# uci-cbcl/esm-efficient

Measured on AMD Instinct MI355X. Metric: residues/sec ESM2-650M fwd, 50k packed tokens; % bf16 MFMA peak; 1/2/4/8 GPU, higher is better.
Workload: dtype bf16

## Files before the change

esm-efficient_amd/csrc/forward.hip:

```cpp
#include "launch.h"

using namespace esme;

namespace {

#define ESME_TRY(call) do { if (const int rc_ = (call)) return rc_; } while (0)

enum Mode { FAST, HALF, EXACT };
const char* const kWho[] = {"forward", "forward_half", "forward_exact"};
constexpr float kLog2e = 1.4426950408889634f;

struct Arena {
    char* base;
    int64_t off;
    char* take(int64_t bytes) {
        const int64_t o = off;
        off += (bytes + 255) & ~int64_t(255);
        return base ? base + o : nullptr;
    }
};

struct Ws {
    char* xs;
    char* h;
// ... 83 lines not shown
    layout(mode, m, T, &w, workspace);
    const int Ep = m->phys_dim, E = m->embed_dim, H = m->heads, dp = m->head_pad;
    const int64_t Ea = (int64_t)H * dp;
    const int nblk = esme_hip_gemm_stats_blocks(T, Ep);
    const bool rot_fused = m->rotary && !m->qk_norm && (dp == 16 || dp == 32 || dp == 64) && Ea % 32 == 0;
    const bool qk_pair = half && m->half_qk_pair != 0;
    if (qk_pair && (m->qk_norm || !(dp == 16 || dp == 32 || dp == 64) || Ea % 128 != 0))
        ESME_FAIL(ESME_ERR_UNSUPPORTED, "forward_half: q/k pairs cover blocks without q/k LayerNorm, head dim 16 / 32 / 64, heads * head_pad a multiple of 128");
    const int ext = half && m->half_ext_n > 0 ? 64 : 0;
    const int64_t lo_off = (int64_t)Ep + ext;
    void* const xs = half ? w.xs : x;
    const int64_t ldxs = half ? 2 * (int64_t)Ep + ext : ldx;
    const int Kf = Ep + ext;
    const bool qp = m->attn_q_prescale && m->rotary && (dp == 64 || dp == 32) && Ea % 64 == 0 && (rot_fused || m->qk_norm);
    const float qs = m->softmax_scale * kLog2e;
    esme_attn_opts_t aopts{(int)sizeof(esme_attn_opts_t), 0, 0, 8.0f, 1, nullptr, qp ? 1 : 0, half ? 1 : 0};
    if (m->n_layers > 0) ESME_TRY(sequence_order(cu_lens, B, w.order, stream, &aopts.seq_order));
    const float* stats = w.sums;
    int stats_nblk = 1;
    if (half)
        ESME_TRY(esme_hip_stream_operand_guarded((const float*)x, ldx, xs, ldxs, lo_off, 1, m->layers[0].ps_attn, ext ? m->half_ext_sel : nullptr, m->half_ext_n,
                                                 ext ? Ep : 0, w.sums, m->half_col_absmax, T, Ep, stream));
    else if (m->n_layers > 0)
        ESME_TRY(esme_hip_row_sums(x, ldx, T, Ep, w.sums, stream));
    auto folded = [&](esme_gemm_fusion_t& f, const float* c1, const float* c2) {
        if (half) { f.f16 = 1; f.overflow_flag = m->half_overflow_flag; }
        ln_fields(f, m, stats, stats_nblk, c1, c2);
    };
    auto residual = [&](const void* a, int64_t lda, const void* wt, const void* bias, int K, float* stats_out, const float* s_in, const float* s_out, int guard_row) {
        esme_gemm_fusion_t f{};
        f.stats_out = stats_out;
        if (half) {
            f.f16 = 1; f.pair_off = lo_off;
            if (ext) { f.ext_sel = m->half_ext_sel; f.ext_n = m->half_ext_n; f.ext_off = Ep; }
            f.pair_scale_in = s_in; f.pair_scale_out = s_out;
            if (m->half_col_absmax) f.col_absmax = m->half_col_absmax + (int64_t)guard_row * Ep;
        }
        return esme_hip_gemm_bf16_fused(a, lda, wt, bias, xs, ldxs, xs, ldxs, T, Ep, K, ESME_EPI_RESIDUAL, m->alpha, &f, stream);
    };
    for (int i = 0; i < m->n_layers; ++i) {
        const esme_layer_weights_t& L = m->layers[i];
        esme_gemm_fusion_t fu{};
        folded(fu, L.qkv_c1, L.qkv_c2);
        char* q = w.qkv; char* k = w.qkv + Ea * 2; char* v = w.qkv + 2 * Ea * 2;
        if (qk_pair && L.half_qk_pair) {
            fu.pair_off = 3 * Ea; fu.pair_cols = (int)(2 * Ea);
            if (m->rotary) rotary_fields(fu, m, m->cos32, m->sin32, pos);
            ESME_TRY(esme_hip_gemm_bf16_fused(xs, ldxs, L.qkv_w, nullptr, nullptr, 0, w.qkv, 5 * Ea, T, (int)(3 * Ea), Kf, ESME_EPI_NONE, 1.0f, &fu, stream));
            ESME_TRY(esme_hip_attn_varlen_fwd_qkpair_f16(q, k, v, 5 * Ea, 3 * Ea, w.attn, Ea, cu_lens, B, T, H, dp, max_len, m->softmax_scale, aopts.seq_order, stream));
        } else {
            uint32_t* const gq = half && m->half_qk_sumsq ? m->half_qk_sumsq + (int64_t)i * 2 * H : nullptr;
            if (rot_fused) { rotary_fields(fu, m, m->cos, m->sin, pos); fu.qk_sumsq = gq; }
            if (qp && rot_fused) { fu.q_scale = qs; fu.q_cols = (int)Ea; }
            ESME_TRY(esme_hip_gemm_bf16_fused(xs, ldxs, L.qkv_w, nullptr, nullptr, 0, w.qkv, 3 * Ea, T, (int)(3 * Ea), Kf, ESME_EPI_NONE, 1.0f, &fu, stream));
            if (m->qk_norm) {
                if (!half) ESME_TRY(esme_hip_qk_norm_rotary_scaled(q, k, 3 * Ea, L.lnq_w, L.lnk_w, L.lnq_b, L.lnk_b, m->ln_eps, m->cos, m->sin, pos, T, H, dp, m->table_len, qp ? qs : 1.0f, stream));
                else if (qp) ESME_TRY(esme_hip_qk_norm_rotary_f16_scaled(q, k, 3 * Ea, L.lnq_w, L.lnk_w, L.lnq_b, L.lnk_b, m->ln_eps, m->cos, m->sin, pos, T, H, dp, m->table_len, qs, gq, stream));
                else ESME_TRY(esme_hip_qk_norm_rotary_f16_guarded(q, k, 3 * Ea, L.lnq_w, L.lnk_w, L.lnq_b, L.lnk_b, m->ln_eps, m->cos, m->sin, pos, T, H, dp, m->table_len, gq, stream));
            } else if (m->rotary && !rot_fused) {
                ESME_TRY((half ? esme_hip_rotary_varlen_f16 : esme_hip_rotary_varlen)(q, k, 3 * Ea, m->cos, m->sin, pos, T, H, dp, m->table_len, stream));
            }
            ESME_TRY(esme_hip_attn_varlen_fwd_opts(q, k, v, 3 * Ea, w.attn, Ea, cu_lens, B, T, H, dp, max_len, m->softmax_scale, &aopts, stream));
        }
        ESME_TRY(residual(w.attn, Ea, L.out_w, L.out_b, (int)Ea, w.part_b, L.ps_attn_inv, L.ps_ffn, 2 * i + 1));
        stats = w.part_b; stats_nblk = nblk;
        esme_gemm_fusion_t fup{};
        folded(fup, L.up_c1, L.up_c2);
        ESME_TRY(esme_hip_gemm_bf16_fused(xs, ldxs, L.up_w, nullptr, nullptr, 0, w.mid, m->ffn_dim, T, m->swiglu ? 2 * m->ffn_dim : m->ffn_dim, Kf,
                                          m->swiglu ? ESME_EPI_SWIGLU : ESME_EPI_GELU, 1.0f, &fup, stream));
// ... 3 lines not shown
    if (half)
        return esme_hip_layernorm_split_checked(xs, ldxs, 2, lo_off, m->final_ln_w, m->final_ln_b, pair, ld_pair, Ep, rep32, ld_rep, T, E, m->ln_eps, m->half_overflow_flag, stream);
    ESME_TRY(esme_hip_layernorm(x, ldx, m->final_ln_w, m->final_ln_b, x, ldx, T, E, m->ln_eps, stream));
    if (!logits) return ESME_OK;
    ESME_CHECK_ARG(m->head_dense_w && m->head_ln_w && m->head_final_w && m->vocab > 0 && ld_logits >= m->vocab, "forward: LM head weights missing");
    ESME_TRY(esme_hip_gemm_bf16(x, ldx, m->head_dense_w, m->head_dense_b, nullptr, 0, w.head, Ep, T, Ep, Ep, ESME_EPI_GELU, 1.0f, stream));
    ESME_TRY(esme_hip_layernorm(w.head, Ep, m->head_ln_w, m->head_ln_b, w.head, Ep, T, E, m->ln_eps, stream));
    return esme_hip_gemm_bf16(w.head, Ep, m->head_final_w, m->head_final_b, nullptr, 0, logits, ld_logits, T, m->vocab, Ep, ESME_EPI_NONE, 1.0f, stream);
}

}

extern "C" int64_t esme_hip_forward_workspace_bytes(const esme_model_desc_t* m, int64_t T) { return workspace_bytes(FAST, m, T); }
extern "C" int64_t esme_hip_forward_half_workspace_bytes(const esme_model_desc_t* m, int64_t T) { return workspace_bytes(HALF, m, T); }
extern "C" int64_t esme_hip_forward_exact_workspace_bytes(const esme_model_desc_t* m, int64_t T) { return workspace_bytes(EXACT, m, T); }

extern "C" int esme_hip_forward(const esme_model_desc_t* m, void* x, int64_t ldx, const int32_t* cu_lens, int B, int64_t T,
                                int max_len, const int32_t* pos, void* workspace, int64_t ws_bytes, void* logits,
                                int64_t ld_logits, void* stream) {
    ESME_PROLOGUE(FAST, m, x, ldx, cu_lens, B, T, max_len, pos, workspace, ws_bytes, nullptr, 0);
    return forward_folded(FAST, m, x, ldx, cu_lens, B, T, max_len, pos, workspace, logits, ld_logits, nullptr, 0, nullptr, 0, stream);
}

extern "C" int esme_hip_forward_half(const esme_model_desc_t* m, const float* x32, int64_t ld32, const int32_t* cu_lens, int B, int64_t T,
                                     int max_len, const int32_t* pos, void* workspace, int64_t ws_bytes, void* pair, int64_t ld_pair,
                                     float* rep32, int64_t ld_rep, void* stream) {
    ESME_PROLOGUE(HALF, m, x32, ld32, cu_lens, B, T, max_len, pos, workspace, ws_bytes, pair, ld_pair);
    return forward_folded(HALF, m, const_cast<float*>(x32), ld32, cu_lens, B, T, max_len, pos, workspace, nullptr, 0, pair, ld_pair, rep32, ld_rep, stream);
}

// ... 44 lines not shown
```

esm-efficient_amd/esme/_hip.py:

```python
from __future__ import annotations

import ctypes
import os
import threading
from ctypes import POINTER, Structure, c_char_p, c_float, c_int, c_int64, c_void_p
from typing import Optional

import torch

_LIB_NAME = 'libesme_hip.so'
_LIB_PATH = os.environ.get('ESME_HIP_LIB') or os.path.join(os.path.dirname(os.path.abspath(__file__)), _LIB_NAME)
ABI_VERSION = 10

EPI_NONE, EPI_GELU, EPI_RESIDUAL, EPI_SWIGLU = 0, 1, 2, 3


class GemmFusion(Structure):
    _fields_ = [('ln_partial', c_void_p), ('ln_nblk', c_int), ('ln_dim', c_int), ('ln_eps', c_float), ('ln_c1', c_void_p), ('ln_c2', c_void_p), ('stats_out', c_void_p),
                ('cos', c_void_p), ('sin', c_void_p), ('pos', c_void_p),
                ('head_dim', c_int), ('max_len', c_int), ('rot_cols', c_int), ('resid32', c_void_p), ('ld32', c_int64), ('q_scale', c_float), ('q_cols', c_int),
                ('w_k', c_int), ('pair_off', c_int64), ('c32', c_void_p), ('ldc32', c_int64), ('f16', c_int),
                ('pair_scale_in', c_void_p), ('pair_scale_out', c_void_p),
                ('ext_sel', c_void_p), ('ext_n', c_int), ('ext_off', c_int64), ('pair_cols', c_int), ('overflow_flag', c_void_p),
                ('col_absmax', c_void_p), ('qk_sumsq', c_void_p)]


class GemmOpts(Structure):
# ... 8 lines not shown
class LayerWeights(Structure):
    _fields_ = [(n, c_void_p) for n in ('qkv_w', 'qkv_c1', 'qkv_c2', 'out_w', 'out_b', 'up_w', 'up_c1', 'up_c2',
                                        'down_w', 'down_b', 'lnq_w', 'lnk_w', 'lnq_b', 'lnk_b',
                                        'ps_attn', 'ps_attn_inv', 'ps_ffn', 'ps_ffn_inv',
                                        'ln1_w', 'ln1_b', 'ln2_w', 'ln2_b', 'qkv_b', 'up_b')] + [('half_qk_pair', c_int), ('reserved_', c_int)]


class ModelDesc(Structure):
    _fields_ = ([(n, c_int) for n in ('struct_bytes', 'n_layers', 'embed_dim', 'phys_dim', 'heads', 'head_dim', 'head_pad',
                                      'ffn_dim', 'vocab', 'swiglu', 'rotary', 'qk_norm', 'table_len')]
                + [('ln_eps', c_float), ('alpha', c_float), ('softmax_scale', c_float), ('attn_q_prescale', c_int),
                   ('layers', POINTER(LayerWeights))]
                + [(n, c_void_p) for n in ('final_ln_w', 'final_ln_b', 'head_dense_w', 'head_dense_b', 'head_ln_w',
                                           'head_ln_b', 'head_final_w', 'head_final_b', 'cos', 'sin')]
                + [('half_ext_n', c_int), ('half_ext_sel', c_void_p), ('half_qk_pair', c_int), ('half_overflow_flag', c_void_p),
                   ('cos32', c_void_p), ('sin32', c_void_p), ('half_col_absmax', c_void_p), ('half_qk_sumsq', c_void_p)])


SIGNATURES = {
    'esme_hip_abi_version': (c_int, []),
    'esme_hip_last_error': (c_char_p, []),
    'esme_hip_embed': (c_int, [c_void_p, c_void_p, c_void_p, c_int64, c_int, c_int, c_int, c_int, c_void_p]),
    'esme_hip_embed_positions': (c_int, [c_void_p, c_void_p, c_void_p, c_void_p, c_int, c_void_p, c_int64, c_int, c_int,
                                         c_int, c_int, c_void_p]),
    'esme_hip_seq_positions': (c_int, [c_void_p, c_int, c_int64, c_void_p, c_void_p, c_void_p]),
    'esme_hip_seq_order': (c_int, [c_void_p, c_int, c_void_p, c_void_p]),
    'esme_hip_layernorm': (c_int, [c_void_p, c_int64, c_void_p, c_void_p, c_void_p, c_int64, c_int64, c_int,
                                   c_float, c_void_p]),
    'esme_hip_rotary_varlen': (c_int, [c_void_p, c_void_p, c_int64, c_void_p, c_void_p, c_void_p, c_int64, c_int,
                                       c_int, c_int, c_void_p]),
    'esme_hip_rotary_varlen_f16': (c_int, [c_void_p, c_void_p, c_int64, c_void_p, c_void_p, c_void_p, c_int64, c_int,
# ... 956 lines not shown
```

esm-efficient_amd/esme/attention.py:

```python
from __future__ import annotations

import math
import os
from typing import NamedTuple, Optional

import torch
from torch import nn

from esme import _hip
from esme.nn import GELU, Derived, LayerNorm, Linear, pad_last, pad_rows, version_key
from esme.rotary import RotaryEmbedding

_ATTN_QP = os.environ.get('ESME_ATTN_QP', '1') != '0'


def _q_scale(head_dim: int) -> float:
    import numpy as np
    return float(np.float32(head_dim ** -0.5) * np.float32(1.4426950408889634))


class ForwardContext:
    __slots__ = ('pos', 'cos', 'sin', 'sums', 'part_a', 'part_b', 'fold', 'exact_attn', 'x32', 'order', 'scratch', 'f16', 'xs', 'plan', 'probe', 'ovf', 'cos32', 'sin32', 'guard', 'lora_x', 'observer',
                 'sites', 'fast_site')

    def __init__(self, pos, cos, sin, fold=False, exact_attn=False, f16=False, plan=None, cos32=None, sin32=None, probe=None, ovf=None, guard=None):
        self.pos, self.cos, self.sin = pos, cos, sin
        self.plan = plan
        self.probe = probe
        self.ovf = ovf
        self.guard = guard
        self.cos32, self.sin32 = cos32, sin32
        self.f16 = f16
        self.fold = fold
        self.exact_attn = exact_attn
        self.x32 = None
        self.xs = None
        self.order = None
        self.scratch = {}
        self.sums = None
        self.part_a = None
        self.part_b = None
        self.observer = None
        self.lora_x = None
        self.sites = None
        self.fast_site = None

    def fp32_stream(self, x32, x16, n_layers):
        self.x32 = x32
        self.sites = [{'resid32': x32, 'out': x16}] * (2 * n_layers)

    def pair_stream(self, xs, scales):
        self.xs = xs
        ext = self.plan.ext_sel if self.plan is not None else None
        col = self.guard.col if self.guard is not None else None
        self.sites = sites = []
        for i, ((_, a_inv), (f_rho, f_inv)) in enumerate(scales):
            nxt = scales[i + 1][0][0] if i + 1 < len(scales) else None
            for scale in ((a_inv, f_rho), (f_inv, nxt)):
                sites.append({'resid_pair': xs, 'pair_scale': scale, 'pair_ext': ext, 'col_absmax': col[len(sites) + 1] if col is not None else None})

# ... 313 lines not shown
        guard = ctx.guard if (f16 and ctx is not None) else None
        pair_ext = plan.ext_sel if plan is not None else None
        if stream is None and resid is not None:
            stream = {'resid': resid, 'out': out}
        if qk_pair:
            if self.pre_layernorm or d not in (16, 32, 64) or E % 128 != 0:
                raise NotImplementedError("precision='half' with q/k pairs covers ESM-2 / ESM-1 blocks with head dim 16 / 32 / 64 and a 128-aligned width")
            wf, _, c1, c2 = self._weights_qkv(True, True, pair_ext)
            qkv = _hip.gemm_fused(x, wf, None, ln=(x_stats, self.embed_dim, self.norm.eps, c1, c2, ctx.ovf), pair_out=True, pair_cols=2 * E,
                                  rot=(ctx.cos32, ctx.sin32, ctx.pos, d, 2 * E) if self.rot_emb is not None else None)
            if ctx.probe is not None:
                ctx.probe.append(_score_bound(qkv[:, :E], qkv[:, E:2 * E], H, d, self.head_dim ** -0.5))
            a = _hip.attn_varlen_qkpair(qkv, cu_lens, max_len, H, d, self.head_dim ** -0.5, order=ctx.order)
            wo, bo = self._weights_out(True)
            return _hip.gemm_fused(a, wo, bo, _hip.EPI_RESIDUAL, alpha=alpha, stats_out=stats_out, **stream)
        if x_stats is not None:
            a_op, wf, c1, c2 = self._qkv_operands(x, x_stats, ctx, lw, f16, pair_ext)
            qkv = _hip.gemm_fused(a_op, wf, None, ln=(x_stats, self.embed_dim, self.norm.eps, c1, c2, ctx.ovf if ctx is not None else None), rot=rot,
                                  q_scale=_q_scale(self.head_dim) if (qp and rot_fusable) else 0.0,
                                  qk_sumsq=guard.qk[self.layer_index] if (guard is not None and rot is not None) else None)
        else:
            if self.padded:
                raise NotImplementedError('padded layouts run the LayerNorm-folded path only')
            qkv = self._qkv_lora_unfused(x, lw, rot)
        if qk_pass:
            _hip.qk_norm_rotary_(qkv[:, :E], qkv[:, E:2 * E], self.layernorm_q.weight, self.layernorm_k.weight,
                                 self.layernorm_q.bias, self.layernorm_k.bias, self.layernorm_q.eps,
                                 ctx.cos, ctx.sin, ctx.pos, H, q_scale=_q_scale(self.head_dim) if qp else 1.0,
                                 qk_sumsq=guard.qk[self.layer_index] if guard is not None else None)
            q, k, v = (qkv[:, i * E:(i + 1) * E].view(T, H, d) for i in range(3))
        else:
# ... 501 lines not shown
        h = ag.layer_norm(x, self.final[0])
        ups, (_, down) = self._ffn_projections()
        if self.final_activation == 'gelu':
            u = torch.nn.functional.gelu(ag.lora_linear(h, ups[0][1], lora_names))
        else:
            u = torch.nn.functional.silu(ag.lora_linear(h, ups[0][1], lora_names)) * ag.lora_linear(h, ups[1][1], lora_names)
        return x + ag.lora_linear(u, down, lora_names) / self.residue_scaling

    def forward(self, x, cu_lens, max_len, lora_names=None, ctx: Optional[ForwardContext] = None,
                inplace: bool = False):
        alpha = 1.0 / self.residue_scaling
        y = x if inplace else torch.empty_like(x)
        T, E = x.shape
        if ctx is not None and ctx.fold and E % 64 == 0:
            if ctx.sums is None:
                ctx.sums = _hip.row_sums(x)
                ctx.part_a = torch.empty(_hip.stats_blocks(T, E), T, 2, dtype=torch.float32, device=x.device)
                ctx.part_b = torch.empty_like(ctx.part_a)
            i = self.self_attn.layer_index
            site = ctx.residual(i, 0, x, y)
            self.self_attn(x, cu_lens, max_len, lora_names, ctx, alpha=alpha, x_stats=ctx.sums, stats_out=ctx.part_b, stream=site)
            self._ffn(y, alpha, site if inplace else ctx.residual(i, 1, y, y), x_stats=ctx.part_b, stats_out=ctx.part_a, lora_names=lora_names, ctx=ctx)
            ctx.sums = ctx.part_a
            return y
        if self.padded:
            raise NotImplementedError('padded layouts need a folding context (ForwardContext(fold=True))')
        self.self_attn(x, cu_lens, max_len, lora_names, ctx, resid=x, alpha=alpha, out=y)
        return self._ffn(y, alpha, {'resid': y, 'out': y}, lora_names=lora_names, ctx=ctx)
```

esm-efficient_amd/esme/cforward.py:

```python
from __future__ import annotations

import ctypes
import operator

import torch

from esme import _hip, attention
from esme._hip import LayerWeights, ModelDesc


def _ptr(t):
    return t.data_ptr() if t is not None else None


_VERSION = operator.attrgetter('_version')
_MODES = {'fast': ('esme_hip_forward', 'esme_hip_forward_workspace_bytes', '_cdesc', 'forward x', torch.bfloat16),
          'half': ('esme_hip_forward_half', 'esme_hip_forward_half_workspace_bytes', '_cdesc16', 'forward x32', torch.float32),
          'exact': ('esme_hip_forward_exact', 'esme_hip_forward_exact_workspace_bytes', '_cdesc_exact', 'forward x32', torch.float32)}


class ModelDescriptor:

    def __init__(self, model, f16: bool = False, plan=None, exact: bool = False):
        self.key = self.signature(model)
# ... 98 lines not shown
        return torch.empty(max(nbytes, 16), dtype=torch.uint8, device=device)
    pool = model.__dict__.setdefault('_cws', {})
    ws = pool.get(key)
    if ws is None or ws.numel() < nbytes:
        if len(pool) >= 8:
            pool.clear()
        ws = pool[key] = torch.empty(max(nbytes, 16), dtype=torch.uint8, device=device)
    return ws


def _refuse_lora(model):
    if getattr(model, 'has_lora', False):
        raise NotImplementedError('the one-call C forward (esme_hip_forward*) has no LoRA adapter path: a model with adapters runs module by module')


def _run(model, mode, x, cu_lens, max_len, pos, cos, sin, pair=None, rep32=None, plan=None, ovf=None, cos32=None, sin32=None, guard=None):
    _refuse_lora(model)
    lib = _hip.load()
    entry, ws_query, attr, x_name, x_dtype = _MODES[mode]
    md = getattr(model, attr, None)
    if md is None or md.key != ModelDescriptor.signature(model) or (mode == 'half' and md.plan is not plan):
        md = ModelDescriptor(model, f16=mode == 'half', plan=plan, exact=mode == 'exact')
        setattr(model, attr, md)
    d = md.desc
    d.cos, d.sin = _ptr(cos), _ptr(sin)
    d.table_len = int(cos.shape[0]) if cos is not None else 0
    if mode == 'half':
        d.half_overflow_flag = _ptr(ovf)
        d.cos32, d.sin32 = _ptr(cos32), _ptr(sin32)
        d.half_col_absmax = _ptr(guard.col) if guard is not None else None
        d.half_qk_sumsq = _ptr(guard.qk) if guard is not None else None
    T, stream, dref = x.shape[0], _hip._stream(), ctypes.byref(d)
    nbytes = int(getattr(lib, ws_query)(dref, T))
    ws = _workspace(model, (x.device.index, stream) if mode == 'fast' else (x.device.index, stream, mode), nbytes, x.device)
    if mode == 'exact' and model.padded:
        ws.zero_()
    xp, cp = _hip._dev(x, x_name, x_dtype), _hip._dev(cu_lens, 'cu_lens', torch.int32)
    out = (None, 0) if mode == 'fast' else (_hip._dev(pair, 'forward pair', torch.bfloat16), pair.stride(0),
                                            _hip._dev(rep32, 'forward rep32', torch.float32), rep32.stride(0))
    _hip._check(getattr(lib, entry)(dref, xp, x.stride(0), cp, cu_lens.numel() - 1, T, int(max_len), _ptr(pos), ws.data_ptr(), ws.numel(), *out, stream), entry)


def forward_layers(model, x, cu_lens, max_len, pos, cos, sin):
    _run(model, 'fast', x, cu_lens, max_len, pos, cos, sin)
    return x


def forward_layers_half(model, x32, cu_lens, max_len, pos, cos, sin, pair, rep32, plan=None, ovf=None, cos32=None, sin32=None, guard=None):
    _run(model, 'half', x32, cu_lens, max_len, pos, cos, sin, pair, rep32, plan, ovf, cos32, sin32, guard)


def forward_layers_exact(model, x32, cu_lens, max_len, pos, cos, sin, pair, rep32):
    _run(model, 'exact', x32, cu_lens, max_len, pos, cos, sin, pair, rep32)
```

esm-efficient_amd/esme/esm.py:

```python
from __future__ import annotations

import math
import os
from typing import List, Optional, Sequence, Tuple

import torch
from torch import nn

from esme import _hip, halfmode
from esme.alphabet import Alphabet, Alphabet3
from esme.attention import FlashTransformerLayer, ForwardContext, padded_head_dim
from esme.head import RobertaLMHead
from esme.embedding import LearnedPositionalEmbedding
from esme.nn import Derived, LayerNorm, bump_epoch, bump_weights_epoch, pad_last, version_key
from esme.qk_observer import dense_blocks

model_names = ['esm2_8m', 'esm2_35m', 'esm2_150m', 'esm2_650m', 'esm2_3b', 'esm2_15b',
               'esmc_300m', 'esmc_600m', 'esm1b', 'esm1v']


def _read_metadata(path: str) -> dict:
    from safetensors import safe_open
    with safe_open(path, framework='pt', device='cpu') as f:
        return dict(f.metadata() or {})
# ... 83 lines not shown
                raise IndexError(f'token id {lo if lo < 0 else hi} is outside the embedding table of {self.embed_tokens.weight.shape[0]} rows')
        return self

    def _embedding_phys(self, tokens, pad_args=None):
        if self.debug_checks:
            self.check_tokens(tokens)
        return _hip.embed(tokens, self._embed_table(),
                          mask_idx=self.alphabet.mask_idx if self.zero_mask_rows else -1,
                          pad_idx=self.alphabet.padding_idx if (tokens.ndim == 2 and self.zero_mask_rows) else -1)

    def _embedding_exact(self, x, tokens, pad_args, pad_indices):
        x32 = torch.empty(x.shape, dtype=torch.float32, device=x.device)
        _hip.residual_f32_(x32, x, 1.0, x, None, init=True)
        return x32

    def _c_forward_ok(self, precision: str = 'fast') -> bool:
        from esme.cforward import ModelDescriptor
        return ModelDescriptor.supported(self, precision)

    half_robust = {'0': False, '1': True}.get(os.environ.get('ESME_HALF_ROBUST', 'auto'), 'auto')
    HALF_CHANNEL_RATIO = 6.0
    HALF_SCORE_BOUND = 32.0
    HALF_QP_BOUND = 16.0
    half_guard = os.environ.get('ESME_HALF_GUARD', '1') != '0'
    half_qp = os.environ.get('ESME_HALF_QP', '1') != '0'
    half_check = 'sync'
    HALF_CALIB_VOCAB = 'all'

    def set_precision(self, mode: str, robust=None, calib=None):
        assert mode in ('fast', 'high', 'half', 'exact'), mode
# ... 69 lines not shown

    def forward_representation(self, tokens, pad_args=None, pad_output=False, pad_indices=None,
                               lora_names=None, layers=None):
        layers = list(layers) if layers else []
        self._check_layers_arg(layers)

        with _hip.stream_scope(self.embed_tokens.weight.device):
            x = self._forward_representation(tokens, pad_args, pad_output, pad_indices, layers, lora_names=lora_names)
            if self.padded:
                E, Ep = self.embed_dim, self.phys_dim
                x = torch.cat([x[..., i * Ep:i * Ep + E] for i in range(x.shape[-1] // Ep)], dim=-1)
            return x

    def _forward_representation(self, tokens, pad_args, pad_output, pad_indices, layers, want_pair=False, lora_names=None, observer=None):
        lora = self._lora_select(lora_names)
        x = self._embedding_phys(tokens, pad_args)
        if pad_args is not None:
            assert tokens.ndim == 1, 'tokens are expected to be unpadded with shape (batch * seq_len)'
            cu_lens, max_len = pad_args
        else:
            assert tokens.ndim == 2, 'tokens are expected to be padded with shape (batch, seq_len, embed_dim)'
            x, pad_indices, cu_lens, max_len = self._unpad(x, tokens)
        if cu_lens.dtype != torch.int32:
            cu_lens = cu_lens.to(torch.int32)
        max_len = int(max_len)

        pad_width = tokens.shape[1] if pad_args is None else max_len
        ctx = self._context(cu_lens, max_len, x.shape[0], x.device)
        if observer is not None:
            ctx.observer = observer(cu_lens, max_len)
        mode = self.precision if self.precision in ('half', 'exact') or (self.precision == 'high' and len(self.layers)) else 'fast'
        x, taps = getattr(self, '_run_' + mode)(x, (tokens, pad_args, pad_indices), cu_lens, max_len, ctx, layers, want_pair, lora)
        return self._finish_representation(x, taps, pad_output, pad_args, pad_indices, cu_lens, pad_width)

    def _one_call(self, ctx, layers, mode) -> bool:
        return bool(self.c_forward and not layers and ctx.observer is None and _hip.TRACE is None and self._c_forward_ok(mode))

    def _final_pair(self, T, device, pair=None):
        alloc = torch.zeros if self.padded else torch.empty
        Ep = self.phys_dim
        return pair if pair is not None else alloc(T, 2 * Ep, dtype=torch.bfloat16, device=device), alloc(T, Ep, dtype=torch.float32, device=device)

    def _run_fast(self, x, embed_args, cu_lens, max_len, ctx, layers, want_pair, lora):
        if self._one_call(ctx, layers, 'fast'):
            from esme import cforward
            return cforward.forward_layers(self, x, cu_lens, max_len, ctx.pos, ctx.cos, ctx.sin), []
        taps, E = [], self.embed_dim
        ctx.order = _hip.seq_order(cu_lens)
        if lora is not None:
            x = self._lora_stream(x, lora, ctx)
        for i, layer in enumerate(self.layers):
            x = layer(x, cu_lens, max_len, lora, ctx, inplace=True)
            if i in layers:
                taps.append(x.clone(memory_format=torch.contiguous_format) if lora is not None else x.clone())
        if ctx.lora_x is not None:
            y = torch.empty(x.shape, dtype=x.dtype, device=x.device)
            self.emb_layer_norm_after(x, out=y)
            return y, taps
        self.emb_layer_norm_after(x[:, :E], out=x[:, :E])
        return x, taps

    def _run_high(self, x, embed_args, cu_lens, max_len, ctx, layers, want_pair, lora):
        assert x.shape[1] % 64 == 0, 'high-precision mode needs a 64-aligned physical width'
# ... 625 lines not shown
```

include/esme_hip.h:

```cpp
#ifndef ESME_HIP_H
#define ESME_HIP_H

#include <stdint.h>

#ifdef __cplusplus
extern "C" {
#endif

#define ESME_HIP_ABI_VERSION 10

enum {
    ESME_OK = 0,
    ESME_ERR_ARG = -1,
    ESME_ERR_UNSUPPORTED = -2,
    ESME_ERR_LAUNCH = -3
};

enum {
    ESME_EPI_NONE = 0,
    ESME_EPI_GELU = 1,
    ESME_EPI_RESIDUAL = 2,
    ESME_EPI_SWIGLU = 3
};

// ... 237 lines not shown
    int rotary;
    int qk_norm;
    int table_len;
    float ln_eps, alpha;
    float softmax_scale;
    int attn_q_prescale;
    const esme_layer_weights_t* layers;
    const void* final_ln_w; const void* final_ln_b;
    const void* head_dense_w; const void* head_dense_b; const void* head_ln_w; const void* head_ln_b;
    const void* head_final_w; const void* head_final_b;
    const void* cos; const void* sin;
    int half_ext_n; const int32_t* half_ext_sel; int half_qk_pair;
    int* half_overflow_flag;
    const float* cos32; const float* sin32;
    uint32_t* half_col_absmax; uint32_t* half_qk_sumsq;
} esme_model_desc_t;

int64_t esme_hip_forward_workspace_bytes(const esme_model_desc_t* model, int64_t T);
int esme_hip_forward(const esme_model_desc_t* model, void* x, int64_t ldx, const int32_t* cu_lens, int B,
                     int64_t T, int max_len, const int32_t* pos, void* workspace, int64_t ws_bytes,
                     void* logits, int64_t ld_logits, void* stream);

int64_t esme_hip_forward_half_workspace_bytes(const esme_model_desc_t* model, int64_t T);
int esme_hip_forward_half(const esme_model_desc_t* model, const float* x32, int64_t ld32, const int32_t* cu_lens, int B,
                          int64_t T, int max_len, const int32_t* pos, void* workspace, int64_t ws_bytes,
                          void* pair, int64_t ld_pair, float* rep32, int64_t ld_rep, void* stream);

int64_t esme_hip_forward_exact_workspace_bytes(const esme_model_desc_t* model, int64_t T);
int esme_hip_forward_exact(const esme_model_desc_t* model, float* x32, int64_t ld32, const int32_t* cu_lens, int B,
                           int64_t T, int max_len, const int32_t* pos, void* workspace, int64_t ws_bytes,
// ... 7 lines not shown
```

Baseline: 804,000.

## Compute layer-0 QKV from a per-vocabulary precomputed table instead of GEMM

Because layer 0's input is a token embedding over a vocabulary of at most 64 entries, the LayerNorm-folded QKV projection of each vocab row is precomputed once into an fp32 table, cached per weight version. A new kernel gathers rows from this table per token and applies rotary and q-prescale to fill the QKV workspace. The forward then skips layer 0's QKV GEMM and the initial row-sum pass. This adds a new entry point, ABI field and cached table, and holds only for unmodified embeddings without LoRA or observers.

```diff
diff --git a/esm-efficient_amd/csrc/forward.hip b/esm-efficient_amd/csrc/forward.hip
--- a/esm-efficient_amd/csrc/forward.hip
+++ b/esm-efficient_amd/csrc/forward.hip
@@ -121,6 +121,8 @@
     const int Kf = Ep + ext;
     const bool qp = m->attn_q_prescale && m->rotary && (dp == 64 || dp == 32) && Ea % 64 == 0 && (rot_fused || m->qk_norm);
     const float qs = m->softmax_scale * kLog2e;
+    const bool qkv0_ready = mode == FAST && m->layer0_qkv_ready != 0;
+    if (qkv0_ready && !(m->n_layers > 0 && rot_fused && (dp == 64 || dp == 32) && Ea % 64 == 0)) return refuse(mode, "layer0_qkv_ready needs a layer that rotates in its QKV epilogue at head dim 64 / 32 (esme_hip_forward_layer0_qkv)");
     esme_attn_opts_t aopts{(int)sizeof(esme_attn_opts_t), 0, 0, 8.0f, 1, nullptr, qp ? 1 : 0, half ? 1 : 0};
     if (m->n_layers > 0) ESME_TRY(sequence_order(cu_lens, B, w.order, stream, &aopts.seq_order));
     const float* stats = w.sums;
@@ -128,7 +130,7 @@
     if (half)
         ESME_TRY(esme_hip_stream_operand_guarded((const float*)x, ldx, xs, ldxs, lo_off, 1, m->layers[0].ps_attn, ext ? m->half_ext_sel : nullptr, m->half_ext_n,
                                                  ext ? Ep : 0, w.sums, m->half_col_absmax, T, Ep, stream));
-    else if (m->n_layers > 0)
+    else if (m->n_layers > 0 && !qkv0_ready)
         ESME_TRY(esme_hip_row_sums(x, ldx, T, Ep, w.sums, stream));
     auto folded = [&](esme_gemm_fusion_t& f, const float* c1, const float* c2) {
         if (half) { f.f16 = 1; f.overflow_flag = m->half_overflow_flag; }
@@ -159,7 +161,8 @@
             uint32_t* const gq = half && m->half_qk_sumsq ? m->half_qk_sumsq + (int64_t)i * 2 * H : nullptr;
             if (rot_fused) { rotary_fields(fu, m, m->cos, m->sin, pos); fu.qk_sumsq = gq; }
             if (qp && rot_fused) { fu.q_scale = qs; fu.q_cols = (int)Ea; }
-            ESME_TRY(esme_hip_gemm_bf16_fused(xs, ldxs, L.qkv_w, nullptr, nullptr, 0, w.qkv, 3 * Ea, T, (int)(3 * Ea), Kf, ESME_EPI_NONE, 1.0f, &fu, stream));
+            if (!(qkv0_ready && i == 0))
+                ESME_TRY(esme_hip_gemm_bf16_fused(xs, ldxs, L.qkv_w, nullptr, nullptr, 0, w.qkv, 3 * Ea, T, (int)(3 * Ea), Kf, ESME_EPI_NONE, 1.0f, &fu, stream));
             if (m->qk_norm) {
                 if (!half) ESME_TRY(esme_hip_qk_norm_rotary_scaled(q, k, 3 * Ea, L.lnq_w, L.lnk_w, L.lnq_b, L.lnk_b, m->ln_eps, m->cos, m->sin, pos, T, H, dp, m->table_len, qp ? qs : 1.0f, stream));
                 else if (qp) ESME_TRY(esme_hip_qk_norm_rotary_f16_scaled(q, k, 3 * Ea, L.lnq_w, L.lnk_w, L.lnq_b, L.lnk_b, m->ln_eps, m->cos, m->sin, pos, T, H, dp, m->table_len, qs, gq, stream));
@@ -193,6 +196,21 @@
 extern "C" int64_t esme_hip_forward_workspace_bytes(const esme_model_desc_t* m, int64_t T) { return workspace_bytes(FAST, m, T); }
 extern "C" int64_t esme_hip_forward_half_workspace_bytes(const esme_model_desc_t* m, int64_t T) { return workspace_bytes(HALF, m, T); }
 extern "C" int64_t esme_hip_forward_exact_workspace_bytes(const esme_model_desc_t* m, int64_t T) { return workspace_bytes(EXACT, m, T); }
+
+extern "C" int esme_hip_forward_layer0_qkv(const esme_model_desc_t* m, int64_t T, int64_t* offset, float* q_scale) {
+    if (!(m && m->struct_bytes == (int)sizeof(esme_model_desc_t))) return refuse(FAST, "descriptor missing or of another ABI");
+    if (!(T >= 0 && offset && q_scale)) return refuse(FAST, "bad sizes or null pointer");
+    const int dp = m->head_pad;
+    const int64_t Ea = (int64_t)m->heads * dp;
+    if (!(m->n_layers > 0 && m->rotary && !m->qk_norm && (dp == 64 || dp == 32) && Ea % 64 == 0))
+        ESME_FAIL(ESME_ERR_UNSUPPORTED, "forward: layer 0's q / k / v come from the caller only where the QKV epilogue rotates (head dim 64 / 32, no q/k LayerNorm)");
+    Ws w;
+    char* const origin = reinterpret_cast<char*>(uintptr_t(4096));
+    layout(FAST, m, T, &w, origin);
+    *offset = w.qkv - origin;
+    *q_scale = m->attn_q_prescale ? m->softmax_scale * kLog2e : 0.f;
+    return ESME_OK;
+}
 
 extern "C" int esme_hip_forward(const esme_model_desc_t* m, void* x, int64_t ldx, const int32_t* cu_lens, int B, int64_t T,
                                 int max_len, const int32_t* pos, void* workspace, int64_t ws_bytes, void* logits,
diff --git a/esm-efficient_amd/csrc/qkv_vocab.hip b/esm-efficient_amd/csrc/qkv_vocab.hip
--- /dev/null
+++ b/esm-efficient_amd/csrc/qkv_vocab.hip
@@ -0,0 +1,189 @@
+#include "common.h"
+#include "launch.h"
+#include "../../include/esme_hip_qkv_vocab.h"
+
+namespace esme {
+
+static constexpr int kVocabRows = 512;
+static constexpr int kVocabUnroll = 4;
+static constexpr int kVocabNtMinMB = 256;
+
+struct VocabArgs {
+    const int64_t* tokens; const int32_t* pos; const float* tab; const u16* cosT; const u16* sinT;
+    u16* out; int64_t ld_out, T;
+    int table_len, N, q_cols, rot_cols, d, V, mask_idx, pad_idx, rows, nt;
+    float q_scale;
+};
+
+int launch_iota(int64_t* ids, int n, hipStream_t s);
+int launch_vocab_pass(const VocabArgs& a, hipStream_t s);
+
+#ifndef ESME_QKV_VOCAB_NO_KERNELS
+__global__ __launch_bounds__(64) void iota_kernel(int64_t* ids, int n) {
+    const int i = blockIdx.x * 64 + threadIdx.x;
+    if (i < n) ids[i] = i;
+}
+
+template <int SLAB>
+__global__ __launch_bounds__(256) void qkv_from_vocab_kernel(const VocabArgs a) {
+    extern __shared__ __attribute__((aligned(16))) float slab[];
+    constexpr int CH = SLAB / 8;
+    constexpr int RPW = 64 / CH;
+    constexpr int RPI = 4 * RPW;
+    const int tid = threadIdx.x, col0 = blockIdx.x * SLAB;
+    for (int i = tid; i < (a.V + 1) * (SLAB / 4); i += 256) {
+        const int r = i / (SLAB / 4), q = i - r * (SLAB / 4);
+        const f32x4 v = *reinterpret_cast<const f32x4*>(a.tab + (int64_t)r * a.N + col0 + 4 * q);
+        *reinterpret_cast<f32x4*>(slab + r * SLAB + (q & 1) * (SLAB / 2) + (q >> 1) * 4) = v;
+    }
+    __syncthreads();
+    const int lane = tid & 63, wave = tid >> 6;
+    const int c = lane % CH, rw = lane / CH;
+    const int col = col0 + c * 8;
+    const int hh = a.d >> 4;
+    const bool rot = col < a.rot_cols, upper = (c & hh) != 0, scale_q = a.q_scale != 0.f && col < a.q_cols;
+    const int cp = c ^ hh, j = c & (hh - 1);
+    const int64_t r0 = (int64_t)blockIdx.y * a.rows;
+    const int64_t r1 = r0 + a.rows < a.T ? r0 + a.rows : a.T;
+    for (int64_t tb = r0 + wave * RPW + rw; tb < r1; tb += (int64_t)kVocabUnroll * RPI) {
+        int row[kVocabUnroll], p[kVocabUnroll];
+#pragma unroll
+        for (int u = 0; u < kVocabUnroll; ++u) {
+            const int64_t t = tb + (int64_t)u * RPI;
+            const int64_t tc = t < r1 ? t : r1 - 1;
+            const int64_t tok = a.tokens[tc];
+            row[u] = (tok < 0 || tok >= a.V || tok == a.mask_idx || tok == a.pad_idx) ? a.V : (int)tok;
+            int pp = rot ? a.pos[tc] : 0;
+            pp = pp < a.table_len ? pp : a.table_len - 1;
+            p[u] = pp > 0 ? pp : 0;
+        }
+        u32x4 cw[kVocabUnroll], sw[kVocabUnroll];
+        if (rot) {
+#pragma unroll
+            for (int u = 0; u < kVocabUnroll; ++u) {
+                cw[u] = *reinterpret_cast<const u32x4*>(a.cosT + (int64_t)p[u] * a.d + j * 8);
+                sw[u] = *reinterpret_cast<const u32x4*>(a.sinT + (int64_t)p[u] * a.d + j * 8);
+            }
+        }
+#pragma unroll
+        for (int u = 0; u < kVocabUnroll; ++u) {
+            const int64_t t = tb + (int64_t)u * RPI;
+            const float* src = slab + row[u] * SLAB;
+            const f32x4 x0 = *reinterpret_cast<const f32x4*>(src + c * 4), x1 = *reinterpret_cast<const f32x4*>(src + SLAB / 2 + c * 4);
+            float o[8] = {x0[0], x0[1], x0[2], x0[3], x1[0], x1[1], x1[2], x1[3]};
+            if (rot) {
+                const f32x4 y0 = *reinterpret_cast<const f32x4*>(src + cp * 4), y1 = *reinterpret_cast<const f32x4*>(src + SLAB / 2 + cp * 4);
+                const float y[8] = {y0[0], y0[1], y0[2], y0[3], y1[0], y1[1], y1[2], y1[3]};
+                float cv[8], sv[8];
+                unpack8(cw[u], cv);
+                unpack8(sw[u], sv);
+#pragma unroll
+                for (int e = 0; e < 8; ++e) {
+                    const float ys = __fmul_rn(y[e], sv[e]);
+                    o[e] = fmaf(o[e], cv[e], upper ? ys : -ys);
+                    if (scale_q) o[e] = __fmul_rn(o[e], a.q_scale);
+                }
+            }
+            if (t < r1) store_stream(reinterpret_cast<u32x4*>(a.out + t * a.ld_out + col), pack8(o), a.nt);
+        }
+    }
+}
+
+template <int SLAB>
+static int launch_vocab(const VocabArgs& a, hipStream_t s) {
+    const int smem = (a.V + 1) * SLAB * 4;
+    auto kern = qkv_from_vocab_kernel<SLAB>;
+    if (smem >= 64 * 1024) {
+        static std::atomic<unsigned long long> done{0ull};
+        if (const int rc = raise_dynamic_lds(done, kern, smem, "qkv_from_vocab")) return rc;
+    }
+    hipLaunchKernelGGL(kern, dim3((unsigned int)(a.N / SLAB), (unsigned int)((a.T + a.rows - 1) / a.rows)), dim3(256), smem, s, a);
+    return check_launch("qkv_from_vocab");
+}
+
+int launch_vocab_pass(const VocabArgs& a, hipStream_t s) {
+    if (a.N % 256 == 0) return launch_vocab<256>(a, s);
+    if (a.N % 128 == 0) return launch_vocab<128>(a, s);
+    return launch_vocab<64>(a, s);
+}
+
+int launch_iota(int64_t* ids, int n, hipStream_t s) {
+    hipLaunchKernelGGL(iota_kernel, dim3((n + 63) / 64), dim3(64), 0, s, ids, n);
+    return check_launch("qkv_vocab_table");
+}
+#endif
+
+}
+
+using namespace esme;
+
+#define ESME_TRY(call) do { if (const int rc_ = (call)) return rc_; } while (0)
+
+static int64_t table_layout(int V, int Ep, int64_t* x_off, int64_t* sums_off) {
+    const int64_t rows = V + 1;
+    const int64_t x = (rows * 8 + 255) & ~int64_t(255), sums = x + ((rows * Ep * 2 + 255) & ~int64_t(255));
+    if (x_off) *x_off = x;
+    if (sums_off) *sums_off = sums;
+    return sums + rows * 2 * 4;
+}
+
+extern "C" int64_t esme_hip_qkv_vocab_table_workspace_bytes(int V, int phys_dim) {
+    if (V <= 0 || phys_dim <= 0) return fail(ESME_ERR_ARG, "qkv_vocab_table: bad sizes");
+    if (V > ESME_HIP_QKV_VOCAB_MAX_V || phys_dim % 64 != 0) return fail(ESME_ERR_UNSUPPORTED, "qkv_vocab_table: V <= 64 and phys_dim a multiple of 64");
+    return table_layout(V, phys_dim, nullptr, nullptr);
+}
+
+extern "C" int esme_hip_qkv_vocab_table(const void* embed_table, int V, int phys_dim, int mask_idx, const void* qkv_w, const float* c1, const float* c2,
+                                        int N, int ln_dim, float ln_eps, void* workspace, int64_t ws_bytes, float* tab, void* stream) {
+    ESME_CHECK_ARG(V > 0 && phys_dim > 0 && N > 0 && ln_dim > 0 && ln_dim <= phys_dim, "qkv_vocab_table: bad sizes");
+    if (V > ESME_HIP_QKV_VOCAB_MAX_V || phys_dim % 64 != 0 || N % 64 != 0) ESME_FAIL(ESME_ERR_UNSUPPORTED, "qkv_vocab_table: V <= 64, phys_dim and N multiples of 64");
+    ESME_CHECK_ARG(embed_table && qkv_w && c1 && c2 && workspace && tab, "qkv_vocab_table: null pointer");
+    int64_t x_off, sums_off;
+    ESME_CHECK_ARG(ws_bytes >= table_layout(V, phys_dim, &x_off, &sums_off) && aligned16(workspace) && aligned16(tab), "qkv_vocab_table: workspace too small or misaligned");
+    int64_t* const ids = (int64_t*)workspace;
+    void* const x = (char*)workspace + x_off;
+    float* const sums = (float*)((char*)workspace + sums_off);
+    const int rows = V + 1;
+    ESME_TRY(launch_iota(ids, rows, (hipStream_t)stream));
+    ESME_TRY(esme_hip_embed(ids, embed_table, x, rows, phys_dim, V, mask_idx, -1, stream));
+    ESME_TRY(esme_hip_row_sums(x, phys_dim, rows, phys_dim, sums, stream));
+    esme_gemm_fusion_t f{};
+    f.ln_partial = sums; f.ln_nblk = 1; f.ln_dim = ln_dim; f.ln_eps = ln_eps; f.ln_c1 = c1; f.ln_c2 = c2;
+    f.c32 = tab; f.ldc32 = N;
+    return esme_hip_gemm_bf16_fused(x, phys_dim, qkv_w, nullptr, nullptr, 0, tab, N, rows, N, phys_dim, ESME_EPI_NONE, 1.0f, &f, stream);
+}
+
+extern "C" int esme_hip_qkv_from_vocab(const int64_t* tokens, const int32_t* pos, const float* tab, const void* cosT, const void* sinT, int table_len,
+                                       float q_scale, void* out, int64_t ld_out, int64_t T, int H, int head_dim, int head_pad, int V, int mask_idx,
+                                       int pad_idx, void* stream) {
+    ESME_CHECK_ARG(T >= 0 && H > 0 && V > 0 && head_dim > 0 && head_dim <= head_pad && table_len > 0, "qkv_from_vocab: bad sizes");
+    if (T == 0) return ESME_OK;
+    if (head_pad != 64 && head_pad != 32) ESME_FAIL(ESME_ERR_UNSUPPORTED, "qkv_from_vocab: head dims 64 and 32 (what the fused rotary epilogue scales q for)");
+    const int64_t Ea = (int64_t)H * head_pad;
+    if (Ea % 64 != 0 || 3 * Ea > 0x7fffffffLL || V > ESME_HIP_QKV_VOCAB_MAX_V) ESME_FAIL(ESME_ERR_UNSUPPORTED, "qkv_from_vocab: heads * head_pad a multiple of 64, V <= 64");
+    ESME_CHECK_ARG(tokens && pos && tab && cosT && sinT && out, "qkv_from_vocab: null pointer");
+    ESME_CHECK_ARG(ld_out >= 3 * Ea && ld_out % 8 == 0 && aligned16(out) && aligned16(tab) && aligned16(cosT) && aligned16(sinT), "qkv_from_vocab: ld_out < 3 * heads * head_pad, ld_out % 8 != 0 or misaligned");
+    VocabArgs a{tokens, pos, tab, (const u16*)cosT, (const u16*)sinT, (u16*)out, ld_out, T,
+                table_len, (int)(3 * Ea), (int)Ea, (int)(2 * Ea), head_pad, V, mask_idx, pad_idx, kVocabRows, 0, q_scale};
+    while ((T + a.rows - 1) / a.rows > 65535) a.rows *= 2;
+    a.nt = (double)T * a.N * 2.0 > kVocabNtMinMB * 1048576.0;
+    return launch_vocab_pass(a, (hipStream_t)stream);
+}
+
+extern "C" int esme_hip_forward_tokens(const esme_model_desc_t* m, const int64_t* tokens, const void* embed_table, int V, int mask_idx, int pad_idx,
+                                       const float* tab, void* x, int64_t ldx, const int32_t* cu_lens, int B, int64_t T, int max_len,
+                                       const int32_t* pos, void* workspace, int64_t ws_bytes, void* logits, int64_t ld_logits, void* stream) {
+    int64_t off = 0;
+    float qs = 0.f;
+    ESME_TRY(esme_hip_forward_layer0_qkv(m, T, &off, &qs));
+    if (T == 0) return ESME_OK;
+    ESME_CHECK_ARG(tokens && embed_table && tab && x && workspace && pos && m->cos && m->sin, "forward_tokens: null pointer");
+    ESME_CHECK_ARG(ldx == m->phys_dim, "forward_tokens: x must be contiguous (ldx == phys_dim): the embedding is written into it");
+    ESME_CHECK_ARG(ws_bytes >= esme_hip_forward_workspace_bytes(m, T) && aligned16(workspace), "forward_tokens: workspace too small or misaligned");
+    ESME_TRY(esme_hip_embed(tokens, embed_table, x, T, m->phys_dim, V, mask_idx, pad_idx, stream));
+    ESME_TRY(esme_hip_qkv_from_vocab(tokens, pos, tab, m->cos, m->sin, m->table_len, qs, (char*)workspace + off, 3 * (int64_t)m->heads * m->head_pad, T,
+                                     m->heads, m->head_dim, m->head_pad, V, mask_idx, pad_idx, stream));
+    esme_model_desc_t ready = *m;
+    ready.layer0_qkv_ready = 1;
+    return esme_hip_forward(&ready, x, ldx, cu_lens, B, T, max_len, pos, workspace, ws_bytes, logits, ld_logits, stream);
+}
diff --git a/esm-efficient_amd/esme/_hip.py b/esm-efficient_amd/esme/_hip.py
--- a/esm-efficient_amd/esme/_hip.py
+++ b/esm-efficient_amd/esme/_hip.py
@@ -10,7 +10,7 @@
 
 _LIB_NAME = 'libesme_hip.so'
 _LIB_PATH = os.environ.get('ESME_HIP_LIB') or os.path.join(os.path.dirname(os.path.abspath(__file__)), _LIB_NAME)
-ABI_VERSION = 10
+ABI_VERSION = 11
 
 EPI_NONE, EPI_GELU, EPI_RESIDUAL, EPI_SWIGLU = 0, 1, 2, 3
 
@@ -49,7 +49,8 @@
                 + [(n, c_void_p) for n in ('final_ln_w', 'final_ln_b', 'head_dense_w', 'head_dense_b', 'head_ln_w',
                                            'head_ln_b', 'head_final_w', 'head_final_b', 'cos', 'sin')]
                 + [('half_ext_n', c_int), ('half_ext_sel', c_void_p), ('half_qk_pair', c_int), ('half_overflow_flag', c_void_p),
-                   ('cos32', c_void_p), ('sin32', c_void_p), ('half_col_absmax', c_void_p), ('half_qk_sumsq', c_void_p)])
+                   ('cos32', c_void_p), ('sin32', c_void_p), ('half_col_absmax', c_void_p), ('half_qk_sumsq', c_void_p),
+                   ('layer0_qkv_ready', c_int), ('reserved_', c_int)])
 
 
 SIGNATURES = {
diff --git a/esm-efficient_amd/esme/_hip_qkv_vocab.py b/esm-efficient_amd/esme/_hip_qkv_vocab.py
--- /dev/null
+++ b/esm-efficient_amd/esme/_hip_qkv_vocab.py
@@ -0,0 +1,70 @@
+from __future__ import annotations
+
+import ctypes
+from ctypes import POINTER, c_float, c_int, c_int64, c_void_p
+
+import torch
+
+from esme import _hip
+
+MAX_V = 64
+
+SIGNATURES = {
+    'esme_hip_qkv_vocab_table_workspace_bytes': (c_int64, [c_int, c_int]),
+    'esme_hip_qkv_vocab_table': (c_int, [c_void_p, c_int, c_int, c_int, c_void_p, c_void_p, c_void_p, c_int, c_int, c_float, c_void_p, c_int64,
+                                         c_void_p, c_void_p]),
+    'esme_hip_qkv_from_vocab': (c_int, [c_void_p, c_void_p, c_void_p, c_void_p, c_void_p, c_int, c_float, c_void_p, c_int64, c_int64, c_int, c_int,
+                                        c_int, c_int, c_int, c_int, c_void_p]),
+    'esme_hip_forward_layer0_qkv': (c_int, [POINTER(_hip.ModelDesc), c_int64, POINTER(c_int64), POINTER(c_float)]),
+    'esme_hip_forward_tokens': (c_int, [POINTER(_hip.ModelDesc), c_void_p, c_void_p, c_int, c_int, c_int, c_void_p, c_void_p, c_int64, c_void_p, c_int,
+                                        c_int64, c_int, c_void_p, c_void_p, c_int64, c_void_p, c_int64, c_void_p]),
+}
+
+
+def bind(lib) -> None:
+    for name, (res, args) in SIGNATURES.items():
+        fn = getattr(lib, name)
+        fn.restype, fn.argtypes = res, args
+
+
+def _lib():
+    lib = _hip.load()
+    if isinstance(lib, ctypes.CDLL):
+        bind(lib)
+    return lib
+
+
+def vocab_table(embed_table: torch.Tensor, mask_idx: int, qkv_w: torch.Tensor, c1: torch.Tensor, c2: torch.Tensor, ln_dim: int, ln_eps: float) -> torch.Tensor:
+    V, Ep = embed_table.shape
+    N = qkv_w.shape[0]
+    if not (embed_table.is_contiguous() and qkv_w.is_contiguous() and qkv_w.shape[1] == Ep):
+        raise ValueError('vocab_table: contiguous (V, phys_dim) table and (N, phys_dim) weight expected')
+    lib = _lib()
+    nbytes = lib.esme_hip_qkv_vocab_table_workspace_bytes(int(V), int(Ep))
+    if nbytes < 0:
+        _hip._check(nbytes, 'esme_hip_qkv_vocab_table_workspace_bytes')
+    ws = torch.empty(int(nbytes), dtype=torch.uint8, device=embed_table.device)
+    tab = torch.empty(V + 1, N, dtype=torch.float32, device=embed_table.device)
+    with _hip._Traced('qkv_vocab_table', (V, N, Ep)):
+        _hip._check(lib.esme_hip_qkv_vocab_table(_hip._dev(embed_table, 'vocab_table embedding', torch.bfloat16), int(V), int(Ep), int(mask_idx),
+                                                 _hip._dev(qkv_w, 'vocab_table weight', torch.bfloat16), _hip._dev(c1, 'vocab_table c1', torch.float32),
+                                                 _hip._dev(c2, 'vocab_table c2', torch.float32), int(N), int(ln_dim), float(ln_eps),
+                                                 ws.data_ptr(), ws.numel(), tab.data_ptr(), _hip._stream()), 'esme_hip_qkv_vocab_table')
+    return tab
+
+
+def qkv_from_vocab(tokens: torch.Tensor, pos: torch.Tensor, tab: torch.Tensor, cos: torch.Tensor, sin: torch.Tensor, heads: int, head_dim: int,
+                   q_scale: float = 0.0, mask_idx: int = -1, pad_idx: int = -1, out: torch.Tensor = None) -> torch.Tensor:
+    T, V, N = tokens.numel(), tab.shape[0] - 1, tab.shape[1]
+    head_pad = N // (3 * heads)
+    if tokens.dim() != 1 or not tokens.is_contiguous() or pos.numel() != T or not tab.is_contiguous() or cos.shape != sin.shape or cos.shape[1] != head_pad:
+        raise ValueError('qkv_from_vocab: contiguous 1-D tokens, one position per token, a contiguous table and (table_len, head_pad) cos / sin expected')
+    if out is None:
+        out = torch.empty(T, N, dtype=torch.bfloat16, device=tokens.device)
+    op, ld = _hip._rows2d(out, 'qkv_from_vocab out')
+    with _hip._Traced('qkv_from_vocab', (T, N, V)):
+        _hip._check(_lib().esme_hip_qkv_from_vocab(_hip._dev(tokens, 'qkv_from_vocab tokens', torch.int64), _hip._dev(pos, 'qkv_from_vocab pos', torch.int32),
+                                                   _hip._dev(tab, 'qkv_from_vocab table', torch.float32), _hip._dev(cos, 'qkv_from_vocab cos', torch.bfloat16),
+                                                   _hip._dev(sin, 'qkv_from_vocab sin', torch.bfloat16), int(cos.shape[0]), float(q_scale), op, ld, T, int(heads),
+                                                   int(head_dim), int(head_pad), int(V), int(mask_idx), int(pad_idx), _hip._stream()), 'esme_hip_qkv_from_vocab')
+    return out
diff --git a/esm-efficient_amd/esme/attention.py b/esm-efficient_amd/esme/attention.py
--- a/esm-efficient_amd/esme/attention.py
+++ b/esm-efficient_amd/esme/attention.py
@@ -21,7 +21,7 @@
 
 class ForwardContext:
     __slots__ = ('pos', 'cos', 'sin', 'sums', 'part_a', 'part_b', 'fold', 'exact_attn', 'x32', 'order', 'scratch', 'f16', 'xs', 'plan', 'probe', 'ovf', 'cos32', 'sin32', 'guard', 'lora_x', 'observer',
-                 'sites', 'fast_site')
+                 'sites', 'fast_site', 'qkv0_tab', 'from_tokens', 'qkv0')
 
     def __init__(self, pos, cos, sin, fold=False, exact_attn=False, f16=False, plan=None, cos32=None, sin32=None, probe=None, ovf=None, guard=None):
         self.pos, self.cos, self.sin = pos, cos, sin
@@ -44,6 +44,9 @@
         self.lora_x = None
         self.sites = None
         self.fast_site = None
+        self.qkv0_tab = None
+        self.from_tokens = False
+        self.qkv0 = None
 
     def fp32_stream(self, x32, x16, n_layers):
         self.x32 = x32
@@ -387,7 +390,9 @@
             a = _hip.attn_varlen_qkpair(qkv, cu_lens, max_len, H, d, self.head_dim ** -0.5, order=ctx.order)
             wo, bo = self._weights_out(True)
             return _hip.gemm_fused(a, wo, bo, _hip.EPI_RESIDUAL, alpha=alpha, stats_out=stats_out, **stream)
-        if x_stats is not None:
+        if x_stats is not None and ctx is not None and ctx.qkv0 is not None and self.layer_index == 0:
+            qkv = ctx.qkv0
+        elif x_stats is not None:
             a_op, wf, c1, c2 = self._qkv_operands(x, x_stats, ctx, lw, f16, pair_ext)
             qkv = _hip.gemm_fused(a_op, wf, None, ln=(x_stats, self.embed_dim, self.norm.eps, c1, c2, ctx.ovf if ctx is not None else None), rot=rot,
                                   q_scale=_q_scale(self.head_dim) if (qp and rot_fusable) else 0.0,
@@ -919,9 +924,9 @@
         T, E = x.shape
         if ctx is not None and ctx.fold and E % 64 == 0:
             if ctx.sums is None:
-                ctx.sums = _hip.row_sums(x)
                 ctx.part_a = torch.empty(_hip.stats_blocks(T, E), T, 2, dtype=torch.float32, device=x.device)
                 ctx.part_b = torch.empty_like(ctx.part_a)
+                ctx.sums = _hip.row_sums(x) if ctx.qkv0 is None else ctx.part_a
             i = self.self_attn.layer_index
             site = ctx.residual(i, 0, x, y)
             self.self_attn(x, cu_lens, max_len, lora_names, ctx, alpha=alpha, x_stats=ctx.sums, stats_out=ctx.part_b, stream=site)
diff --git a/esm-efficient_amd/esme/cforward.py b/esm-efficient_amd/esme/cforward.py
--- a/esm-efficient_amd/esme/cforward.py
+++ b/esm-efficient_amd/esme/cforward.py
@@ -136,7 +136,7 @@
         raise NotImplementedError('the one-call C forward (esme_hip_forward*) has no LoRA adapter path: a model with adapters runs module by module')
 
 
-def _run(model, mode, x, cu_lens, max_len, pos, cos, sin, pair=None, rep32=None, plan=None, ovf=None, cos32=None, sin32=None, guard=None):
+def _run(model, mode, x, cu_lens, max_len, pos, cos, sin, pair=None, rep32=None, plan=None, ovf=None, cos32=None, sin32=None, guard=None, tokens=None):
     _refuse_lora(model)
     lib = _hip.load()
     entry, ws_query, attr, x_name, x_dtype = _MODES[mode]
@@ -160,11 +160,24 @@
     xp, cp = _hip._dev(x, x_name, x_dtype), _hip._dev(cu_lens, 'cu_lens', torch.int32)
     out = (None, 0) if mode == 'fast' else (_hip._dev(pair, 'forward pair', torch.bfloat16), pair.stride(0),
                                             _hip._dev(rep32, 'forward rep32', torch.float32), rep32.stride(0))
+    if tokens is not None:
+        from esme import _hip_qkv_vocab
+        ids, table, mask_idx, tab = tokens
+        _hip_qkv_vocab.bind(lib)
+        _hip._check(lib.esme_hip_forward_tokens(dref, _hip._dev(ids, 'forward tokens', torch.int64), _hip._dev(table, 'forward embedding', torch.bfloat16), int(table.shape[0]),
+                                                int(mask_idx), -1, _hip._dev(tab, 'forward q/k/v table', torch.float32), xp, x.stride(0), cp, cu_lens.numel() - 1, T,
+                                                int(max_len), _ptr(pos), ws.data_ptr(), ws.numel(), *out, stream), 'esme_hip_forward_tokens')
+        return
     _hip._check(getattr(lib, entry)(dref, xp, x.stride(0), cp, cu_lens.numel() - 1, T, int(max_len), _ptr(pos), ws.data_ptr(), ws.numel(), *out, stream), entry)
 
 
 def forward_layers(model, x, cu_lens, max_len, pos, cos, sin):
     _run(model, 'fast', x, cu_lens, max_len, pos, cos, sin)
+    return x
+
+
+def forward_tokens(model, tokens, table, mask_idx, tab, x, cu_lens, max_len, pos, cos, sin):
+    _run(model, 'fast', x, cu_lens, max_len, pos, cos, sin, tokens=(tokens, table, mask_idx, tab))
     return x
 
 
diff --git a/esm-efficient_amd/esme/esm.py b/esm-efficient_amd/esme/esm.py
--- a/esm-efficient_amd/esme/esm.py
+++ b/esm-efficient_amd/esme/esm.py
@@ -7,7 +7,7 @@
 import torch
 from torch import nn
 
-from esme import _hip, halfmode
+from esme import _hip, attention, halfmode
 from esme.alphabet import Alphabet, Alphabet3
 from esme.attention import FlashTransformerLayer, ForwardContext, padded_head_dim
 from esme.head import RobertaLMHead
@@ -121,6 +121,22 @@
         _hip.residual_f32_(x32, x, 1.0, x, None, init=True)
         return x32
 
+    qkv_table = os.environ.get('ESME_NO_QKV_TABLE', '0') != '1'
+
+    def _qkv0_table(self, tokens, pad_args, lora):
+        if not (self.qkv_table and self.precision == 'fast' and len(self.layers) and not torch.is_grad_enabled() and lora is None and not self.has_lora
+                and pad_args is not None and tokens.ndim == 1 and self.fold_layernorm and self.phys_dim % 64 == 0 and type(self)._embedding_phys is ESM2._embedding_phys):
+            return None
+        att = self.layers[0].self_attn
+        if (att.rot_emb is None or att.pre_layernorm or att.head_pad not in (32, 64) or att.attn_dim % 64 or att._q4_qkv is not None or att._has_lora
+                or self.vocab_size > 64 or any(p is not None and p.requires_grad for lin in (att.q, att.k, att.v) for p in (lin.weight, lin.bias))):
+            return None
+        wf, _, c1, c2 = att._weights_qkv(True)
+        table, mask_idx = self._embed_table(), self.alphabet.mask_idx if self.zero_mask_rows else -1
+        from esme import _hip_qkv_vocab
+        return self._derived.get('qkv0_tab', (att._derived.key('fold'), version_key(self.embed_tokens.weight), table.data_ptr(), mask_idx),
+                                 _hip_qkv_vocab.vocab_table, table, mask_idx, wf, c1, c2, self.embed_dim, att.norm.eps)
+
     def _c_forward_ok(self, precision: str = 'fast') -> bool:
         from esme.cforward import ModelDescriptor
         return ModelDescriptor.supported(self, precision)
@@ -220,7 +236,15 @@
 
     def _forward_representation(self, tokens, pad_args, pad_output, pad_indices, layers, want_pair=False, lora_names=None, observer=None):
         lora = self._lora_select(lora_names)
-        x = self._embedding_phys(tokens, pad_args)
+        mode = self.precision if self.precision in ('half', 'exact') or (self.precision == 'high' and len(self.layers)) else 'fast'
+        qkv0_tab = self._qkv0_table(tokens, pad_args, lora) if mode == 'fast' else None
+        from_tokens = bool(qkv0_tab is not None and self.c_forward and not layers and observer is None and _hip.TRACE is None and self._c_forward_ok('fast'))
+        if from_tokens:
+            if self.debug_checks:
+                self.check_tokens(tokens)
+            x = torch.empty(tokens.shape[0], self.phys_dim, dtype=torch.bfloat16, device=self.embed_tokens.weight.device)
+        else:
+            x = self._embedding_phys(tokens, pad_args)
         if pad_args is not None:
             assert tokens.ndim == 1, 'tokens are expected to be unpadded with shape (batch * seq_len)'
             cu_lens, max_len = pad_args
@@ -235,7 +259,7 @@
         ctx = self._context(cu_lens, max_len, x.shape[0], x.device)
         if observer is not None:
             ctx.observer = observer(cu_lens, max_len)
-        mode = self.precision if self.precision in ('half', 'exact') or (self.precision == 'high' and len(self.layers)) else 'fast'
+        ctx.qkv0_tab, ctx.from_tokens = qkv0_tab, from_tokens
         x, taps = getattr(self, '_run_' + mode)(x, (tokens, pad_args, pad_indices), cu_lens, max_len, ctx, layers, want_pair, lora)
         return self._finish_representation(x, taps, pad_output, pad_args, pad_indices, cu_lens, pad_width)
 
@@ -248,11 +272,20 @@
         return pair if pair is not None else alloc(T, 2 * Ep, dtype=torch.bfloat16, device=device), alloc(T, Ep, dtype=torch.float32, device=device)
 
     def _run_fast(self, x, embed_args, cu_lens, max_len, ctx, layers, want_pair, lora):
+        mask_idx = self.alphabet.mask_idx if self.zero_mask_rows else -1
+        if ctx.from_tokens:
+            from esme import cforward
+            return cforward.forward_tokens(self, embed_args[0].contiguous(), self._embed_table(), mask_idx, ctx.qkv0_tab, x, cu_lens, max_len, ctx.pos, ctx.cos, ctx.sin), []
         if self._one_call(ctx, layers, 'fast'):
             from esme import cforward
             return cforward.forward_layers(self, x, cu_lens, max_len, ctx.pos, ctx.cos, ctx.sin), []
         taps, E = [], self.embed_dim
         ctx.order = _hip.seq_order(cu_lens)
+        if ctx.qkv0_tab is not None:
+            from esme import _hip_qkv_vocab
+            att = self.layers[0].self_attn
+            ctx.qkv0 = _hip_qkv_vocab.qkv_from_vocab(embed_args[0], ctx.pos, ctx.qkv0_tab, ctx.cos, ctx.sin, att.num_heads, att.head_dim,
+                                                     q_scale=attention._q_scale(att.head_dim) if attention._ATTN_QP else 0.0, mask_idx=mask_idx)
         if lora is not None:
             x = self._lora_stream(x, lora, ctx)
         for i, layer in enumerate(self.layers):
diff --git a/include/esme_hip.h b/include/esme_hip.h
--- a/include/esme_hip.h
+++ b/include/esme_hip.h
@@ -7,7 +7,7 @@
 extern "C" {
 #endif
 
-#define ESME_HIP_ABI_VERSION 10
+#define ESME_HIP_ABI_VERSION 11
 
 enum {
     ESME_OK = 0,
@@ -275,6 +275,7 @@
     int* half_overflow_flag;
     const float* cos32; const float* sin32;
     uint32_t* half_col_absmax; uint32_t* half_qk_sumsq;
+    int layer0_qkv_ready; int reserved_;
 } esme_model_desc_t;
 
 int64_t esme_hip_forward_workspace_bytes(const esme_model_desc_t* model, int64_t T);
diff --git a/include/esme_hip_qkv_vocab.h b/include/esme_hip_qkv_vocab.h
--- /dev/null
+++ b/include/esme_hip_qkv_vocab.h
@@ -0,0 +1,30 @@
+#ifndef ESME_HIP_QKV_VOCAB_H
+#define ESME_HIP_QKV_VOCAB_H
+
+#include "esme_hip.h"
+
+#ifdef __cplusplus
+extern "C" {
+#endif
+
+#define ESME_HIP_QKV_VOCAB_MAX_V 64
+
+int64_t esme_hip_qkv_vocab_table_workspace_bytes(int V, int phys_dim);
+
+int esme_hip_qkv_vocab_table(const void* embed_table, int V, int phys_dim, int mask_idx, const void* qkv_w, const float* c1, const float* c2,
+                             int N, int ln_dim, float ln_eps, void* workspace, int64_t ws_bytes, float* tab, void* stream);
+
+int esme_hip_qkv_from_vocab(const int64_t* tokens, const int32_t* pos, const float* tab, const void* cos, const void* sin, int table_len,
+                            float q_scale, void* out, int64_t ld_out, int64_t T, int H, int head_dim, int head_pad, int V, int mask_idx,
+                            int pad_idx, void* stream);
+
+int esme_hip_forward_layer0_qkv(const esme_model_desc_t* model, int64_t T, int64_t* offset, float* q_scale);
+
+int esme_hip_forward_tokens(const esme_model_desc_t* model, const int64_t* tokens, const void* embed_table, int V, int mask_idx, int pad_idx,
+                            const float* tab, void* x, int64_t ldx, const int32_t* cu_lens, int B, int64_t T, int max_len,
+                            const int32_t* pos, void* workspace, int64_t ws_bytes, void* logits, int64_t ld_logits, void* stream);
+
+#ifdef __cplusplus
+}
+#endif
+#endif
```

Result: no change. 808,700 (median of 6 runs) (+0.6%).
